# patrickltobing/shallow-wavenet

Measured on AMD Instinct MI355X. Metric: decoded samples/sec (22.05 kHz Laplacian AR decode, whole job), higher is better.
Workload: dtype f32

## Files before the change

shallow_wavenet_amd/csrc/swn_decode_bl6w.hip:

```cpp
#include <type_traits>
#include "swn_decode_bl6_common.hpp"
#include "swn_decode_internal.hpp"

namespace {

using namespace swn_bl6;

constexpr int NG = 256;
constexpr int S = 128;
constexpr int O1 = 128;

template <int LPC_, bool EXT_>
struct Tw {
    static constexpr int LPC = LPC_;
    static constexpr bool EXT = EXT_;
    using Ext = Tw<LPC_, true>;
    static constexpr int NO = 2 + LPC_;
    static constexpr int WN = cmax(1, LPC_) + 1;
    static constexpr int ring_len(int l) { return pow2ceil((1 << l) + 1); }
    static constexpr int ring_off(int l) { int o = 0; for (int i = 0; i < l; ++i) o += ring_len(i) * H; return o; }
    static constexpr int PF = L * 2 * H;
    static constexpr int NZC = 64, NZB = 4;
    static constexpr int o_ring = 0;
    static constexpr int o_hcat = o_ring + ring_off(L);
    static constexpr int o_gp = o_hcat + L * H;
    static constexpr int o_bx = o_gp + 2 * PF;
    static constexpr int o_bd = o_bx + L * 2 * H;
    static constexpr int o_old = o_bd + L * 2 * H;
    static constexpr int o_wup = o_old + 2 * L * 2 * H;
    static constexpr int o_skip = o_wup + 256;
    static constexpr int o_p2 = o_skip + S;
    static constexpr int o_tnz = o_p2 + 4 * NO;
    static constexpr int o_cz = o_tnz + r4(NZB * NZC);
    static constexpr int o_w2 = o_cz + 5 * H;
    static constexpr int o_bias = o_w2 + NO * S + r4(NO);
    static constexpr int o_w1 = o_bias + S + O1;
    static constexpr int o_wl = o_w1 + 8 * O1 * 16;
    static constexpr int o_h0w = o_wl + 8 * NG * 4;
    static constexpr int o_end = o_h0w + 3 * H;
    static constexpr size_t lds_bytes = (size_t)o_end * sizeof(float);
    static constexpr int sess_old = ring_off(L);
    static constexpr int sess_win = sess_old + 2 * L * 2 * H;
    static constexpr int sess_floats = sess_win + r4(WN);
};

__device__ __forceinline__ float sum_quads(float v) {
    v += dpp_f<0x124>(v);
    v += dpp_f<0x128>(v);
    float w = v;
    asm("s_nop 1\n\tv_permlane16_swap_b32 %0, %1" : "+v"(v), "+v"(w));
    v += w;
    w = v;
    asm("s_nop 1\n\tv_permlane32_swap_b32 %0, %1" : "+v"(v), "+v"(w));
    return v + w;
}
__device__ __forceinline__ float quad_sum_by_parity(float own, float other) {
    float s = own + dpp_f<0xB1>(other);
    s += dpp_f<0x4E>(s);
    return s;
}
template <class T, int LAYER>
__device__ __forceinline__ void layer_a(float* lds, const float (&w)[2][16], const int q, const float wj, const int pb, const int po,
                                        const int ta, const float* xr) {
    const int o = ta >> 2, p = ta & 3, pr = p & 1;
    const float e_old = lds[T::o_old + po + LAYER * 2 * H + pr * H + o];
    const float e_gx = fmaf(wj, lds[T::o_gp + pb + LAYER * 2 * H + pr * H + o], lds[T::o_bx + LAYER * 2 * H + pr * H + o]);
    const float e_hp = xr[o];
    float az = 0.f, ac = 0.f;
#pragma unroll
    for (int m = 0; m < 4; ++m) {
        const float4 x = *reinterpret_cast<const float4*>(xr + 16 * p + 4 * m);
        az = fmaf(w[0][4 * m], x.x, az); ac = fmaf(w[1][4 * m], x.x, ac);
        az = fmaf(w[0][4 * m + 1], x.y, az); ac = fmaf(w[1][4 * m + 1], x.y, ac);
        az = fmaf(w[0][4 * m + 2], x.z, az); ac = fmaf(w[1][4 * m + 2], x.z, ac);
        az = fmaf(w[0][4 * m + 3], x.w, az); ac = fmaf(w[1][4 * m + 3], x.w, ac);
    }
    const float sq = quad_sum_by_parity(pr ? ac : az, pr ? az : ac);
    __builtin_amdgcn_sched_barrier(0);
    if (p < 2) {
        const float sa = sq + e_old;
        const float v = e_gx * sa;
        const float e = exp_c(p == 0 ? -v : -2.f * fminf(fabsf(v), 64.f));
        const float r = rcp_c(1.f + e);
        const float res = p == 0 ? r : copysignf((1.f - e) * r, v);
        const float c = dpp_f<0xF5>(res);
        if (p == 0) {
            const float hn = (1.f - res) * c + res * e_hp;
            if (LAYER + 1 < L) {
                constexpr int R2 = T::ring_len(LAYER + 1 < L ? LAYER + 1 : LAYER);
                lds[T::o_ring + T::ring_off(LAYER + 1 < L ? LAYER + 1 : LAYER) + (q & (R2 - 1)) * H + o] = hn;
            }
            lds[T::o_hcat + LAYER * H + o] = hn;
        }
    }
    __builtin_amdgcn_sched_barrier(0);
}

template <class T, int LAYER, int MB = 4>
__device__ __forceinline__ void older_sum(const float* lds, const float (&w)[2][16], const int qn, const int tb, float& az, float& ac) {
    constexpr int dil = 1 << LAYER;
    constexpr int R = T::ring_len(LAYER);
    const int p = tb & 3;
    const float* ring = lds + T::o_ring + T::ring_off(LAYER);
    az = 0.f; ac = 0.f;
#pragma unroll
    for (int m = 0; m < 4; ++m) {
        const float4 x = *reinterpret_cast<const float4*>(ring + ((qn - dil) & (R - 1)) * H + 16 * p + 4 * m);
        float4 w0, w1;
        if (LAYER < L - 1) {
            w0 = make_float4(w[0][4 * m], w[0][4 * m + 1], w[0][4 * m + 2], w[0][4 * m + 3]);
            w1 = make_float4(w[1][4 * m], w[1][4 * m + 1], w[1][4 * m + 2], w[1][4 * m + 3]);
        } else {
            w0 = *reinterpret_cast<const float4*>(lds + T::o_wl + (m * NG + tb) * 4);
            w1 = *reinterpret_cast<const float4*>(lds + T::o_wl + ((4 + m) * NG + tb) * 4);
        }
        az = fmaf(w0.x, x.x, az); ac = fmaf(w1.x, x.x, ac);
        az = fmaf(w0.y, x.y, az); ac = fmaf(w1.y, x.y, ac);
        az = fmaf(w0.z, x.z, az); ac = fmaf(w1.z, x.z, ac);
        az = fmaf(w0.w, x.w, az); ac = fmaf(w1.w, x.w, ac);
        if (MB < 4 && m % MB == MB - 1) __builtin_amdgcn_sched_barrier(0);
    }
    az = sum4(az); ac = sum4(ac);
}
template <class T, int LAYER>
__device__ __forceinline__ void older_store(float* lds, const int qn, const int tb, const float az, const float ac) {
    const int o = tb >> 2, p = tb & 3, pr = p & 1;
    lds[T::o_old + (qn & 1) * (L * 2 * H) + LAYER * 2 * H + pr * H + o] = (p == 0 ? az : ac) + lds[T::o_bd + LAYER * 2 * H + pr * H + o];
}
template <class T, int LAYER, int MB = 4>
__device__ __forceinline__ void older_b(float* lds, const float (&w)[2][16], const int qn, const int tb) {
    float az, ac;
    older_sum<T, LAYER, MB>(lds, w, qn, tb, az, ac);
    if ((tb & 3) < 2) older_store<T, LAYER>(lds, qn, tb, az, ac);
}
template <class T>
__device__ __forceinline__ void older_last_rows(const float* lds, const int qn, const int tb, float4 (&x)[2], float4 (&w)[2][2]) {
    constexpr int LAYER = L - 1, dil = 1 << LAYER, R = T::ring_len(LAYER);
    const float* row = lds + T::o_ring + T::ring_off(LAYER) + ((qn - dil) & (R - 1)) * H + 16 * (tb & 3);
#pragma unroll
    for (int m = 0; m < 2; ++m) {
        x[m] = *reinterpret_cast<const float4*>(row + 4 * m);
        w[m][0] = *reinterpret_cast<const float4*>(lds + T::o_wl + (m * NG + tb) * 4);
        w[m][1] = *reinterpret_cast<const float4*>(lds + T::o_wl + ((4 + m) * NG + tb) * 4);
    }
}
template <class T>
__device__ __forceinline__ void older_last_x(float* lds, const float4 (&xe)[2], const float4 (&we)[2][2], const int qn, const int tb) {
    constexpr int LAYER = L - 1, dil = 1 << LAYER, R = T::ring_len(LAYER);
    const float* row = lds + T::o_ring + T::ring_off(LAYER) + ((qn - dil) & (R - 1)) * H + 16 * (tb & 3);
    float az = 0.f, ac = 0.f;
#pragma unroll
    for (int m = 0; m < 4; ++m) {
        float4 x, w0, w1;
        if (m < 2) { x = xe[m]; w0 = we[m][0]; w1 = we[m][1]; }
        else {
            x = *reinterpret_cast<const float4*>(row + 4 * m);
            w0 = *reinterpret_cast<const float4*>(lds + T::o_wl + (m * NG + tb) * 4);
            w1 = *reinterpret_cast<const float4*>(lds + T::o_wl + ((4 + m) * NG + tb) * 4);
        }
        az = fmaf(w0.x, x.x, az); ac = fmaf(w1.x, x.x, ac);
        az = fmaf(w0.y, x.y, az); ac = fmaf(w1.y, x.y, ac);
        az = fmaf(w0.z, x.z, az); ac = fmaf(w1.z, x.z, ac);
        az = fmaf(w0.w, x.w, az); ac = fmaf(w1.w, x.w, ac);
        if (m == 1) __builtin_amdgcn_sched_barrier(0);
    }
    az = sum4(az); ac = sum4(ac);
    if ((tb & 3) < 2) older_store<T, LAYER>(lds, qn, tb, az, ac);
}
template <int... LS> struct Layers {};
template <class T, int NW, int... LS>
__device__ __forceinline__ void older_bn(Layers<LS...>, float* lds, const float (&w)[NW][2][16], const int qn, const int tb) {
    static_assert(((LS < NW) && ...), "register-resident halves only");
    float az[sizeof...(LS)], ac[sizeof...(LS)];
    int k = 0;
    ((older_sum<T, LS>(lds, w[LS], qn, tb, az[k], ac[k]), ++k), ...);
    if ((tb & 3) < 2) {
        k = 0;
        ((older_store<T, LS>(lds, qn, tb, az[k], ac[k]), ++k), ...);
    }
}

template <class T, int LAYER>
__device__ __forceinline__ void older_rows(const float* lds, const int qn, const int tb, float4 (&x)[4]) {
    constexpr int dil = 1 << LAYER;
    constexpr int R = T::ring_len(LAYER);
    const float* row = lds + T::o_ring + T::ring_off(LAYER) + ((qn - dil) & (R - 1)) * H + 16 * (tb & 3);
#pragma unroll
    for (int m = 0; m < 4; ++m) x[m] = *reinterpret_cast<const float4*>(row + 4 * m);
}
__device__ __forceinline__ void older_sum_x(const float (&w)[2][16], const float4 (&x)[4], float& az, float& ac) {
    az = 0.f; ac = 0.f;
#pragma unroll
    for (int m = 0; m < 4; ++m) {
        az = fmaf(w[0][4 * m], x[m].x, az); ac = fmaf(w[1][4 * m], x[m].x, ac);
        az = fmaf(w[0][4 * m + 1], x[m].y, az); ac = fmaf(w[1][4 * m + 1], x[m].y, ac);
        az = fmaf(w[0][4 * m + 2], x[m].z, az); ac = fmaf(w[1][4 * m + 2], x[m].z, ac);
        az = fmaf(w[0][4 * m + 3], x[m].w, az); ac = fmaf(w[1][4 * m + 3], x[m].w, ac);
    }
    az = sum4(az); ac = sum4(ac);
}
template <class T, int... LS>
__device__ __forceinline__ void older_rows_n(Layers<LS...>, const float* lds, const int qn, const int tb, float4 (&x)[sizeof...(LS)][4]) {
    int k = 0;
    ((older_rows<T, LS>(lds, qn, tb, x[k]), ++k), ...);
}
template <class T, int NW, int... LS>
__device__ __forceinline__ void older_bn_x(Layers<LS...>, float* lds, const float (&w)[NW][2][16], const float4 (&x)[sizeof...(LS)][4],
                                           const int qn, const int tb) {
    static_assert(((LS < NW) && ...), "register-resident halves only");
    float az[sizeof...(LS)], ac[sizeof...(LS)];
    int k = 0;
    ((older_sum_x(w[LS], x[k], az[k], ac[k]), ++k), ...);
    if ((tb & 3) < 2) {
        k = 0;
        ((older_store<T, LS>(lds, qn, tb, az[k], ac[k]), ++k), ...);
    }
}

template <int LAYER>
__device__ __forceinline__ void skip_issue_b(__amdgpu_buffer_rsrc_t wsk2, float4 (&wsl)[8], const int tb, const unsigned step0) {
    const int r = tb >> 2, hp = tb & 3;
#pragma unroll
    for (int ps = 0; ps < 2; ++ps)
#pragma unroll
        for (int mm = 0; mm < 4; ++mm)
            wsl[ps * 4 + mm] = buf_ld4(wsk2, (unsigned)((r + 64 * ps) * 4 + hp) * 16u, (unsigned)((LAYER * 4 + mm) * S) * 64u + step0);
}
template <class T, int LAYER>
__device__ __forceinline__ void skip_roll_b(const float* lds, __amdgpu_buffer_rsrc_t wsk2, float4 (&wsl)[8], float (&sacc)[2], const int tb,
                                            const unsigned step0) {
    static_assert(LAYER >= 1 && LAYER < L, "slice LAYER - 1 in flight, slice LAYER to request");
    const int r = tb >> 2, hp = tb & 3;
    float4 xs[4];
#pragma unroll
    for (int mm = 0; mm < 4; ++mm) xs[mm] = *reinterpret_cast<const float4*>(lds + T::o_hcat + (LAYER - 1) * H + 16 * mm + 4 * hp);
#pragma unroll
    for (int mm = 0; mm < 4; ++mm) {
#pragma unroll
        for (int ps = 0; ps < 2; ++ps) {
            const float4 x = xs[mm], w = wsl[ps * 4 + mm];
            sacc[ps] = fmaf(w.x, x.x, sacc[ps]); sacc[ps] = fmaf(w.y, x.y, sacc[ps]);
            sacc[ps] = fmaf(w.z, x.z, sacc[ps]); sacc[ps] = fmaf(w.w, x.w, sacc[ps]);
        }
        __builtin_amdgcn_sched_barrier(0);
#pragma unroll
        for (int ps = 0; ps < 2; ++ps)
            wsl[ps * 4 + mm] = buf_ld4(wsk2, (unsigned)((r + 64 * ps) * 4 + hp) * 16u, (unsigned)((LAYER * 4 + mm) * S) * 64u + step0);
        __builtin_amdgcn_sched_barrier(0);
    }
    asm volatile("" : "+v"(sacc[0]), "+v"(sacc[1]));
}
template <class T>
__device__ __forceinline__ void skip_last_b(float* lds, const float4 (&wsl)[8], const float (&sacc)[2], const int tb) {
    const int r = tb >> 2, hp = tb & 3;
    float part[2][4];
#pragma unroll
    for (int mm = 0; mm < 4; ++mm) {
        const float4 x = *reinterpret_cast<const float4*>(lds + T::o_hcat + (L - 1) * H + 16 * mm + 4 * hp);
#pragma unroll
        for (int ps = 0; ps < 2; ++ps) {
            const float4 w = wsl[ps * 4 + mm];
            part[ps][mm] = fmaf(w.w, x.w, fmaf(w.z, x.z, fmaf(w.y, x.y, w.x * x.x)));
        }
    }
    float s[2];
#pragma unroll
    for (int ps = 0; ps < 2; ++ps) s[ps] = sacc[ps] + ((part[ps][0] + part[ps][1]) + (part[ps][2] + part[ps][3]));
    const float t0 = s[0] + dpp_f<0xB1>(s[0]), t1 = s[1] + dpp_f<0xB1>(s[1]);
    const float v = (hp < 2 ? t0 : t1) + dpp_f<0x4E>(hp < 2 ? t1 : t0);
    if ((hp & 1) == 0) lds[T::o_skip + r + 32 * hp] = fmaxf(v, 0.f);
}

using OlderMerged = Layers<3, 4>;
using OlderOut1 = Layers<0, 1, 2>;

template <class T, bool GA, bool STREAM, bool POOL = false>
__device__ __forceinline__ void decode_body(const Bl6Args& a, float* lds) {
    constexpr bool EXT = T::EXT;
    static_assert(!STREAM || EXT, "streamed chunks run the extended mode");
    constexpr bool grpA = GA;
    const int tid = threadIdx.x, b = POOL ? 0 : blockIdx.x;
    __builtin_assume(GA ? tid < NG : tid >= NG);
    const int tg = tid & (NG - 1);
    const float* __restrict__ P = a.P;
    const int U = a.U;
    const int s0 = STREAM ? a.step0 : 0;
    const bool resume = STREAM && a.resume;
    const int fb0 = STREAM ? s0 / U : 0;

    for (int e = tid; e < T::o_end; e += NT) lds[e] = 0.f;
    __syncthreads();
    for (int e = tid; e < L * 2 * H; e += NT) {
        lds[T::o_bx + e] = P[a.y.bx + e];
        const float bd = P[a.y.bd + e];
        lds[T::o_bd + e] = bd;
        lds[T::o_old + e] = bd;
    }
    for (int e = tid; e < U; e += NT) lds[T::o_wup + e] = P[a.y.wup + e];
    for (int e = tid; e < H; e += NT) lds[T::o_cz + e] = P[a.y.cb + e];
    for (int e = tid; e < S; e += NT) lds[T::o_bias + e] = P[a.y.bsk + e];
    for (int e = tid; e < O1; e += NT) lds[T::o_bias + S + e] = P[a.y.b1 + e];
    for (int e = tid; e < 2 * H; e += NT) { lds[T::o_cz + H + e] = P[a.y.cv + e]; lds[T::o_cz + 3 * H + e] = P[a.y.cc + e]; }
    for (int e = tid; e < T::NO * S; e += NT) lds[T::o_w2 + e] = P[a.y.w2 + (size_t)(e / S) * r4(S) + (e % S)];
    for (int e = tid; e < T::NO; e += NT) lds[T::o_w2 + T::NO * S + e] = P[a.y.b2 + e];
    for (int e = tid; e < 8 * O1 * 16; e += NT) lds[T::o_w1 + e] = P[a.y.w12 + e];
    const __amdgpu_buffer_rsrc_t condr =
        make_rsrc(a.cond + (size_t)b * a.Tf * a.N, (unsigned)((size_t)a.Tf * a.N * sizeof(float)));
    auto load_frame = [&](int fr) {
        float* dst = lds + T::o_gp + (fr & 1) * T::PF;
#pragma unroll
        for (int it = 0; it < (T::PF / 4 + NT - 1) / NT; ++it) {
            const int e4 = it * NT + tid;
            if (e4 < T::PF / 4)
                *reinterpret_cast<float4*>(dst + 4 * e4) =
                    buf_ld4(condr, (unsigned)tid * 16u, (unsigned)(fr * a.N * 4 + it * NT * 16));
        }
    };
    for (int fr = fb0; fr < fb0 + 2 && fr < a.Tf; ++fr) load_frame(fr);
    constexpr int NWR = grpA ? L : L - 1;
    float wreg[NWR][2][16];
    {
        const int o = tg >> 2, p = tg & 3, k = grpA ? 1 : 0;
#pragma unroll
        for (int l = 0; l < L; ++l)
#pragma unroll
            for (int r = 0; r < 2; ++r) {
                const float4* src = reinterpret_cast<const float4*>(P + a.y.wd + (((size_t)l * 2 * H + o + r * H) * 2 + k) * H + 16 * p);
#pragma unroll
                for (int v = 0; v < 4; ++v) {
                    const float4 t = src[v];
                    if (l == L - 1 && !grpA) {
                        *reinterpret_cast<float4*>(lds + T::o_wl + ((r * 4 + v) * NG + tg) * 4) = t;
                    } else {
                        float (&wr)[16] = wreg[l < NWR ? l : 0][r];
                        wr[4 * v] = t.x; wr[4 * v + 1] = t.y; wr[4 * v + 2] = t.z; wr[4 * v + 3] = t.w;
                    }
                }
            }
    }
    __syncthreads();
    const float* sess_b = STREAM ? a.sess + (size_t)b * T::sess_floats : nullptr;
    int tcp = tid;
    asm volatile("" : "+v"(tcp));
    if (resume) {
        for (int e = tcp; e < T::ring_off(L); e += NT) lds[T::o_ring + e] = sess_b[e];
        for (int e = tcp; e < 2 * L * 2 * H; e += NT) lds[T::o_old + e] = sess_b[T::sess_old + e];
        __syncthreads();
    }

    int fb = fb0, tb0 = fb0 * U;
    const int n_pro = RF;
    auto cond_taps = [&](int q, float& wj, int& pb) {
        const int t0 = q - RF;
        const int tlo = t0 < 0 ? 0 : t0;
        if (tlo >= tb0 + U) {
            fb += 1; tb0 += U;
            if (fb + 1 < a.Tf) load_frame(fb + 1);
        }
        int rel = tlo - tb0;
        int fsel = fb;
        if (rel >= U) { rel -= U; fsel = fb + 1; }
        rel = rel < U ? rel : U - 1;
        wj = lds[T::o_wup + rel];
        pb = (fsel & 1) * T::PF;
    };

    auto input_seed = [&](int q) {
        if (tid < H) {
            const int o = tid;
            float acc = c_b;
#pragma unroll
            for (int k = 0; k < 2; ++k) {
                const int r = q - (1 - k);
                if (r >= 0) acc += fmaf(k ? c_v1 : c_v0, 0.f, k ? c_c1 : c_c0);
            }
            lds[T::o_ring + (q & 1) * H + o] = ssign(acc);
        }
    };
    float win[T::WN];
#pragma unroll
    for (int k = 0; k < T::WN; ++k) win[k] = 0.f;
    if (EXT && a.seed) win[T::WN - 1] = reinterpret_cast<const float*>(a.seed)[b];
    if (resume) {
#pragma unroll
        for (int k = 0; k < T::WN; ++k) win[k] = sess_b[T::sess_win + k];
    }
    const int wv = __builtin_amdgcn_readfirstlane(tg >> 6);
    float kcb = 0.f, kv0 = 0.f, kv1 = 0.f, kc0 = 0.f, kc1 = 0.f;
    if (grpA) { const int o = tg & (H - 1); kcb = c_b; kv0 = c_v0; kv1 = c_v1; kc0 = c_c0; kc1 = c_c1; }
    auto h0_row = [&](int qn) -> int {
        return wv == 0 ? T::o_ring + (qn & 1) * H : T::o_h0w + (wv - 1) * H;
    };
    auto input_gen = [&](int row) {
        if constexpr (grpA) {
            float acc = kcb;
            acc += fmaf(kv0, win[T::WN - 2], kc0);
            acc += fmaf(kv1, win[T::WN - 1], kc1);
            lds[row + (tg & (H - 1))] = ssign(acc);
            lds_fence_compiler();
        }
    };
    float e_next = 0.f;
    auto noise_load = [&](int c) {
        const int step = c * T::NZC + tid - 64;
        if (step < a.n_steps) e_next = a.noise[(size_t)b * a.n_steps + step];
    };
    auto noise_chunk = [&](int c) {
        if (grpA && tid >= 64 && tid < 128) {
            const int k = tid - 64, step = c * T::NZC + k;
            if (step < a.n_steps) {
                const float e = EXT ? swn_noise_laplace_at(a.nz, b, step, s0 + step, 0, a.n_steps, 1) : e_next;
                const float sg = (e > 0.f) ? 1.f : ((e < 0.f) ? -1.f : 0.f);
                lds[T::o_tnz + (c & (T::NZB - 1)) * T::NZC + k] = sg * log1pf(-2.f * fabsf(e));
            }
            if (!EXT) noise_load(c + 1);
        }
    };
    if (!EXT && grpA && tid >= 64 && tid < 128) noise_load(0);
    noise_chunk(0);
    noise_chunk(1);

    const __amdgpu_buffer_rsrc_t wsk2 = make_rsrc(P + a.y.wsk2, (unsigned)(L * S * 64 * sizeof(float)));

#ifdef SWN_STAMP
    unsigned long long tw[9] = {0, 0, 0, 0, 0, 0, 0, 0, 0}, tv[6] = {0, 0, 0, 0, 0, 0}, tstep = 0, tlast = 0, tbeg = 0;
#define SWN_BAR(k) { tw[k] += __builtin_amdgcn_s_memtime() - tlast; lds_barrier(); tlast = __builtin_amdgcn_s_memtime(); }
#define SWN_WAIT_STAMP(k) { asm volatile("" :: "v"(wsl[0].x)); tv[k] += __builtin_amdgcn_s_memtime() - tlast; }
#define SWN_PRE(k) { tw[k] += __builtin_amdgcn_s_memtime() - tlast; asm volatile("s_waitcnt lgkmcnt(0)" ::: "memory"); }
#define SWN_BAR_KEEP(k, N) { lds_barrier_keep<N>(); tlast = __builtin_amdgcn_s_memtime(); }
#else
#define SWN_BAR(k) lds_barrier();
#define SWN_WAIT_STAMP(k)
#define SWN_PRE(k)
#define SWN_BAR_KEEP(k, N) lds_barrier_keep<N>();
#endif
#define SWN_PHASE_WORK(LAYER, GEN, X0)                                                                                \
    if constexpr (grpA) layer_a<T, LAYER>(lds, wreg[LAYER], q, wj, pb, po, tg,                                         \
                                          LAYER == 0 ? (X0) : lds + T::o_ring + T::ring_off(LAYER) +                   \
                                                                  (q & (T::ring_len(LAYER) - 1)) * H);                 \
    else {                                                                                                             \
        if (GEN) {    \
                      \
                      \
            if (LAYER == 0) skip_issue_b<0>(wsk2, wsl, tg, step0);                                                     \
            else { SWN_WAIT_STAMP(LAYER > 0 ? LAYER - 1 : 0) skip_roll_b<T, (LAYER > 0 ? LAYER : 1)>(lds, wsk2, wsl, sacc, tg, step0); } \
            __builtin_amdgcn_sched_barrier(0);                                                                         \
        }                                                                                                              \
        if (!(GEN)) older_b<T, LAYER>(lds, wreg[LAYER < NWR ? LAYER : 0], q + 1, tg);                                  \
        else if (LAYER == 0) older_bn<T>(OlderMerged{}, lds, wreg, q + 1, tg);                                         \
        __builtin_amdgcn_sched_barrier(0);                                                                             \
    }
#define SWN_PHASE(LAYER, GEN, X0) SWN_PHASE_WORK(LAYER, GEN, X0) if (GEN) { SWN_BAR(LAYER) } else lds_barrier();

#pragma unroll 1
    for (int q = resume ? n_pro : 0; q < n_pro; ++q) {
        float wj; int pb;
        float4 wsl[8]; float sacc[2]; const unsigned step0 = 0;
        cond_taps(q, wj, pb);
        const int po = (q & 1) * (L * 2 * H);
        input_seed(q);
        lds_barrier();
        const float* x0 = lds + T::o_ring + (q & 1) * H;
        SWN_PHASE(0, false, x0) SWN_PHASE(1, false, x0) SWN_PHASE(2, false, x0) SWN_PHASE(3, false, x0)
        SWN_PHASE(4, false, x0) SWN_PHASE(5, false, x0)
        (void)wsl; (void)sacc; (void)step0;
    }

    int rel_c = s0 - fb0 * U;
    bool fill_c = false;
    float wj_c = 0.f;
    int pb_c = 0, po_c = 0, x0_c = 0;
    auto taps_ahead = [&](int qn) {
        wj_c = lds[T::o_wup + rel_c];
        pb_c = (fb & 1) * T::PF;
        po_c = (qn & 1) * (L * 2 * H);
        x0_c = h0_row(qn);
        asm volatile("" : "+s"(pb_c), "+s"(po_c), "+s"(x0_c));
    };
    auto frame_advance = [&]() {
        rel_c += 1;
        const bool cross = rel_c >= U;
        if (cross) { rel_c = 0; fb += 1; }
        fill_c = cross && fb + 1 < a.Tf;
    };
    if constexpr (grpA) taps_ahead(RF + s0);
    input_gen(x0_c);
#ifdef SWN_STAMP
    tlast = tbeg = __builtin_amdgcn_s_memtime();
#endif
    auto gen_step = [&](const int i) __attribute__((always_inline)) {
        const int q = RF + s0 + i;
        const float wj = wj_c;
        const int pb = pb_c, po = po_c;
        if constexpr (grpA) {
            if (fill_c) load_frame(fb + 1);
        }
        float4 wsl[8];
        float sacc[2] = {0.f, 0.f};
        if constexpr (!grpA) {
            const float bs0 = lds[T::o_bias + (tg >> 2)], bs1 = lds[T::o_bias + (tg >> 2) + 64];
            if ((tg & 3) == 0) { sacc[0] = bs0; sacc[1] = bs1; }
        }
        unsigned step0 = 0;
        asm volatile("" : "+s"(step0));
        const float* x0 = lds + x0_c;
        SWN_PHASE(0, true, x0) SWN_PHASE(1, true, x0) SWN_PHASE(2, true, x0) SWN_PHASE(3, true, x0)
        SWN_PHASE(4, true, x0)
        constexpr bool EARLY5 = T::LPC == 0;
        float4 xl[2], wl[2][2];
        SWN_PHASE_WORK(5, true, x0)
        if constexpr (grpA && EARLY5) {
            SWN_PRE(5)
            lds_fence_compiler();
            __builtin_amdgcn_sched_barrier(0);
            older_last_rows<T>(lds, q + 1, tg + (int)step0, xl, wl);
            __builtin_amdgcn_sched_barrier(0);
            SWN_BAR_KEEP(5, 6)
        } else {
            SWN_BAR(5)
        }
        constexpr bool ROLL1 = T::LPC == 0;
        float4 xo[3][4];
        float4 w1e[2][2];
        if constexpr (!grpA) {
            SWN_WAIT_STAMP(5) skip_last_b<T>(lds, wsl, sacc, tg);
            SWN_PRE(6)
            lds_fence_compiler();
            __builtin_amdgcn_sched_barrier(0);
            older_rows_n<T>(OlderOut1{}, lds, q + 1, tg, xo);
            __builtin_amdgcn_sched_barrier(0);
            SWN_BAR_KEEP(6, 12)
        } else {
            if constexpr (EARLY5) older_last_x<T>(lds, xl, wl, q + 1, tg + (int)step0);
            else older_b<T, L - 1, 2>(lds, wreg[L - 1], q + 1, tg + (int)step0);
            if constexpr (ROLL1) {
                SWN_PRE(6)
                lds_fence_compiler();
                __builtin_amdgcn_sched_barrier(0);
#pragma unroll
                for (int mm = 0; mm < 2; ++mm)
#pragma unroll
                    for (int r = 0; r < 2; ++r)
                        w1e[mm][r] = *reinterpret_cast<const float4*>(lds + T::o_w1 + ((mm * O1 + (tg >> 2) + 64 * r) * 4 + (tg & 3)) * 4);
                __builtin_amdgcn_sched_barrier(0);
                SWN_BAR_KEEP(6, 4)
            } else {
                SWN_BAR(6)
            }
        }
        if constexpr (grpA) {
            const int hr = tg >> 2, hp = tg & 3;
            float a0 = 0.f, a1 = 0.f, b0 = 0.f, b1 = 0.f;
            auto X = [&](int mm) { return *reinterpret_cast<const float4*>(lds + T::o_skip + 16 * mm + 4 * hp); };
            auto W = [&](int mm, int r) { return *reinterpret_cast<const float4*>(lds + T::o_w1 + ((mm * O1 + hr + 64 * r) * 4 + hp) * 4); };
            auto fma8 = [&](int mm, const float4& x0, const float4& w0, const float4& w1) {
                float& acc = (mm & 1) ? a1 : a0;
                float& bcc = (mm & 1) ? b1 : b0;
                acc = fmaf(w0.x, x0.x, acc); acc = fmaf(w0.y, x0.y, acc); acc = fmaf(w0.z, x0.z, acc); acc = fmaf(w0.w, x0.w, acc);
                bcc = fmaf(w1.x, x0.x, bcc); bcc = fmaf(w1.y, x0.y, bcc); bcc = fmaf(w1.z, x0.z, bcc); bcc = fmaf(w1.w, x0.w, bcc);
            };
            float e_b1[2] = {0.f, 0.f}, e_w2[2] = {0.f, 0.f}, e_b2 = 0.f;
            const int e_kc = hp < T::NO ? hp : T::NO - 1;
            if constexpr (ROLL1) {
                static_assert(T::NO <= 4, "one round of out_2 rows");
                float4 xr[3] = {X(0), X(1), X(2)};
                __builtin_amdgcn_sched_barrier(0);
#pragma unroll
                for (int mm = 0; mm < 8; ++mm) {
                    fma8(mm, xr[mm % 3], w1e[mm % 2][0], w1e[mm % 2][1]);
                    __builtin_amdgcn_sched_barrier(0);
                    if (mm + 2 < 8) { w1e[mm % 2][0] = W(mm + 2, 0); w1e[mm % 2][1] = W(mm + 2, 1); }
                    if (mm + 3 < 8) xr[mm % 3] = X(mm + 3);
                    if (mm == 5) {
                        e_b1[0] = lds[T::o_bias + S + hr]; e_b1[1] = lds[T::o_bias + S + hr + 64];
                        e_w2[0] = lds[T::o_w2 + e_kc * S + hr]; e_w2[1] = lds[T::o_w2 + e_kc * S + hr + 64];
                    }
                    if (mm == 6) e_b2 = lds[T::o_w2 + T::NO * S + e_kc];
                    __builtin_amdgcn_sched_barrier(0);
                }
            } else {
#pragma unroll
                for (int mm = 0; mm < 8; ++mm) {
                    fma8(mm, X(mm), W(mm, 0), W(mm, 1));
                    if ((mm & 3) == 3) __builtin_amdgcn_sched_barrier(0);
                }
            }
            const float v = sum4(a0 + a1), u = sum4(b0 + b1);
            if constexpr (ROLL1) {
                const float o1a = fmaxf(v + e_b1[0], 0.f), o1b = fmaxf(u + e_b1[1], 0.f);
                const float pz = sum_quads(fmaf(e_w2[1], o1b, fmaf(e_w2[0], o1a, tg < 4 ? e_b2 : 0.f)));
                if ((tg & 63) < 4 && hp < T::NO) lds[T::o_p2 + 4 * hp + wv] = pz;
            } else {
                const float o1a = fmaxf(v + lds[T::o_bias + S + hr], 0.f), o1b = fmaxf(u + lds[T::o_bias + S + hr + 64], 0.f);
#pragma unroll
                for (int j = 0; j < (T::NO + 3) / 4; ++j) {
                    const int k = hp + 4 * j, kc = k < T::NO ? k : T::NO - 1;
                    const float* w2 = lds + T::o_w2 + kc * S;
                    const float b2 = lds[T::o_w2 + T::NO * S + kc];
                    const float pz = sum_quads(fmaf(w2[hr + 64], o1b, fmaf(w2[hr], o1a, tg < 4 ? b2 : 0.f)));
                    if ((tg & 63) < 4 && k < T::NO) lds[T::o_p2 + 4 * k + wv] = pz;
                }
            }
        } else {
            older_bn_x<T>(OlderOut1{}, lds, wreg, xo, q + 1, tg);
        }
        SWN_BAR(7)
        if constexpr (grpA) {
            const int ln = tg & 63;
            float tz = 0.f;
            if constexpr (!EXT) tz = lds[T::o_tnz + (i & (T::NZB * T::NZC - 1))];
            float fv = 0.f;
            if (a.forced) fv = reinterpret_cast<const float*>(a.forced)[(size_t)b * a.n_steps + i];
            const float4 pz = *reinterpret_cast<const float4*>(lds + T::o_p2 + 4 * (ln < T::NO ? ln : T::NO - 1));
            __builtin_amdgcn_sched_barrier(0);
            frame_advance();
            taps_ahead(q + 1);
            __builtin_amdgcn_sched_barrier(0);
            const float acc = (pz.x + pz.y) + (pz.z + pz.w);
            float o2[T::NO];
#pragma unroll
            for (int k = 0; k < T::NO; ++k) o2[k] = __builtin_bit_cast(float, __builtin_amdgcn_readlane(__builtin_bit_cast(int, acc), k));
            float sv;
            {
#pragma clang fp contract(off)
                const float mu = o2[0];
                const float bsc = sigm(o2[1]);
                float lpv = 0.f;
#pragma unroll
                for (int k = 0; k < T::LPC; ++k) lpv += o2[2 + T::LPC - 1 - k] * win[T::WN - T::LPC + k];
                const float t = bsc * (EXT ? lds[T::o_tnz + ((i >> 6) & (T::NZB - 1)) * T::NZC + (i & (T::NZC - 1))] : tz);
                sv = (T::LPC > 0) ? (lpv + mu) - t : mu - t;
                sv = fminf(fmaxf(sv, -1.f), 1.f);
                float fd = a.forced ? fv : sv;
                asm volatile("" : "+v"(fd));
#pragma unroll
                for (int k = 0; k + 1 < T::WN; ++k) win[k] = win[k + 1];
                win[T::WN - 1] = fd;
            }
            if (i + 1 < a.n_steps) input_gen(x0_c);
            __builtin_amdgcn_sched_barrier(0);
            if (tid == 0) reinterpret_cast<float*>(a.out)[(size_t)b * a.n_steps + (size_t)i] = sv;
            if (HEADS_ON && a.heads && wv == 0 && ln < T::NO) a.heads[((size_t)b * a.n_steps + i) * T::NO + ln] = acc;
        }
#ifdef SWN_STAMP
        if constexpr (grpA) tw[8] += __builtin_amdgcn_s_memtime() - tlast;
#endif
    };
#pragma unroll 1
    for (int i0 = 0; i0 < a.n_steps; i0 += T::NZC) {
        noise_chunk((i0 >> 6) + 2);
        const int iend = i0 + T::NZC < a.n_steps ? i0 + T::NZC : a.n_steps;
#pragma unroll 1
        for (int i = i0; i < iend; ++i) gen_step(i);
    }
#ifdef SWN_STAMP
    { const unsigned long long tn = __builtin_amdgcn_s_memtime(); tw[0] += tn - tlast; tstep = tn - tbeg; }
#endif
    if constexpr (STREAM) {
        __syncthreads();
        float* so = a.sess + (size_t)b * T::sess_floats;
        tcp = tid;
        asm volatile("" : "+v"(tcp));
        for (int e = tcp; e < T::ring_off(L); e += NT) so[e] = lds[T::o_ring + e];
        for (int e = tcp; e < 2 * L * 2 * H; e += NT) so[T::sess_old + e] = lds[T::o_old + e];
        if (tid == 0) {
#pragma unroll
            for (int k = 0; k < T::WN; ++k) so[T::sess_win + k] = win[k];
        }
    }
#undef SWN_PHASE
#undef SWN_PHASE_WORK
#undef SWN_BAR
#undef SWN_WAIT_STAMP
#undef SWN_PRE
#undef SWN_BAR_KEEP
#ifdef SWN_STAMP
    if ((tid == 0 || tid == 64 || tid == NG) && b == 0 && a.heads) {
        float* h = a.heads + (tid == 0 ? 0 : tid == 64 ? 30 : 10);
        for (int k = 0; k < 9; ++k) h[k] = (float)((double)tw[k] / (double)a.n_steps);
        if (tid == 0) h[9] = (float)((double)tstep / (double)a.n_steps);
        else if (tid == NG) for (int k = 0; k < 6; ++k) h[10 + k] = (float)((double)tv[k] / (double)a.n_steps);
    }
#endif
}

template <class T, bool STREAM = false>
__global__ __launch_bounds__(NT) void decode_bl6w_kernel(const Bl6Args a) {
    extern __shared__ __attribute__((aligned(16))) float lds[];
    if (threadIdx.x < NG) decode_body<T, true, STREAM>(a, lds);
    else decode_body<T, false, STREAM>(a, lds);
}

template <class T, bool MODELS = false>
__global__ __launch_bounds__(NT) void decode_bl6w_pool_kernel(
    const typename std::conditional<MODELS, Bl6PoolModelsArgs, Bl6PoolArgs>::type p) {
    extern __shared__ __attribute__((aligned(16))) float lds[];
    static_assert(T::EXT, "pools run the extended mode");
    Bl6Args a = p.c;
    if constexpr (MODELS) a.P = swn_pool_model(p.m);
    if (!swn_pool_entry_args(a, p.t, 1, 1, T::NO)) return;
    a.sess += (size_t)swn_pool_slot(p.t) * T::sess_floats;
    if (threadIdx.x < NG) decode_body<T, true, true, true>(a, lds);
    else decode_body<T, false, true, true>(a, lds);
}

bool bl6w_applies(const SwnGeom& g) {
    return g.bl6 && g.U <= 256 && g.U >= 2 && !g.audio_in && g.kind == SWN_KIND_LAPLACE && g.S == 128 && g.O1 == 128 &&
           g.seg == 1 && (g.lpc == 0 || g.lpc == 4);
}

template <class F>
int with_tw(const SwnGeom& g, F&& f) {
    if (!bl6w_applies(g)) return SWN_E_UNSUPPORTED;
    if (g.lpc == 0) return f(Tw<0, false>{});
    return f(Tw<4, false>{});
}

}

int swn_decode_bl6w_run(const SwnDecodeCall& c) {
    const hipStream_t st = c.hip_stream;
    if (c.pool) {
        Bl6PoolModelsArgs p;
        fill_args(p.c, c);
        p.t = *c.pool;
        if (c.models) p.m = *c.models;
        return with_tw(c.g, [&](auto tw) {
            using T = typename decltype(tw)::Ext;
            if (c.models)
                return launch_kernel(decode_bl6w_pool_kernel<T, true>, T::lds_bytes, c.batch, p, st, "swn_decode_pool_chunk_models(bl6w)");
            const Bl6PoolArgs& p1 = p;
            return launch_kernel(decode_bl6w_pool_kernel<T>, T::lds_bytes, c.batch, p1, st, "swn_decode_pool_chunk(bl6w)");
        });
    }
    Bl6Args a;
    fill_args(a, c);
    return with_tw(c.g, [&](auto t) {
        using T = decltype(t);
        using X = typename T::Ext;
        static_assert(T::lds_bytes <= 160 * 1024 && X::lds_bytes <= 160 * 1024, "LDS budget");
        if (c.stream) return launch_kernel(decode_bl6w_kernel<X, true>, X::lds_bytes, a.B, a, st, "swn_decode(bl6w)");
        if (wants_ext(a)) return launch_kernel(decode_bl6w_kernel<X>, X::lds_bytes, a.B, a, st, "swn_decode(bl6w)");
        return launch_kernel(decode_bl6w_kernel<T>, T::lds_bytes, a.B, a, st, "swn_decode(bl6w)");
    });
}

size_t swn_decode_bl6w_session_floats(const SwnGeom& g) {
    int n = 0;
    with_tw(g, [&](auto t) { n = decltype(t)::sess_floats; return SWN_OK; });
    return (size_t)n;
}
```

Baseline: 395,200.

## Rotate per-step side work behind layer-0 LDS loads and keep one skip slice resident

In the non-extended, LPC==0 path, group A now issues the first quads of layer-0 LDS input loads and then runs the per-step side work while those loads are in flight. That side work is the noise-chunk refresh, the frame load and a deferred buffer store of the previous step's output and heads. The step loop is flattened so noise refresh happens inside the step. Group B can optionally keep the first or last skip-weight slice resident in registers so one global reload per step is skipped; this is controlled by a macro whose default is off. The aim is to hide LDS and store latency on the serial decode critical path, at the cost of more registers and output writes that lag by one step.

```diff
diff --git a/shallow_wavenet_amd/csrc/swn_decode_bl6w.hip b/shallow_wavenet_amd/csrc/swn_decode_bl6w.hip
--- a/shallow_wavenet_amd/csrc/swn_decode_bl6w.hip
+++ b/shallow_wavenet_amd/csrc/swn_decode_bl6w.hip
@@ -1,6 +1,13 @@
 #include <type_traits>
 #include "swn_decode_bl6_common.hpp"
 #include "swn_decode_internal.hpp"
+
+#ifndef SWN_RES_SLICE
+#define SWN_RES_SLICE 0
+#endif
+#ifndef SWN_ROTATE
+#define SWN_ROTATE 1
+#endif
 
 namespace {
 
@@ -59,17 +66,31 @@
     s += dpp_f<0x4E>(s);
     return s;
 }
-template <class T, int LAYER>
+struct NoWork { __device__ __forceinline__ void operator()() const {} };
+template <class T, int LAYER, int NQ = 2, class BEHIND = NoWork>
 __device__ __forceinline__ void layer_a(float* lds, const float (&w)[2][16], const int q, const float wj, const int pb, const int po,
-                                        const int ta, const float* xr) {
+                                        const int ta, const float* xr, BEHIND&& behind = NoWork{}) {
+    constexpr bool ROT = !std::is_same<typename std::decay<BEHIND>::type, NoWork>::value;
     const int o = ta >> 2, p = ta & 3, pr = p & 1;
     const float e_old = lds[T::o_old + po + LAYER * 2 * H + pr * H + o];
-    const float e_gx = fmaf(wj, lds[T::o_gp + pb + LAYER * 2 * H + pr * H + o], lds[T::o_bx + LAYER * 2 * H + pr * H + o]);
+    const float g_gp = lds[T::o_gp + pb + LAYER * 2 * H + pr * H + o], g_bx = lds[T::o_bx + LAYER * 2 * H + pr * H + o];
     const float e_hp = xr[o];
+    static_assert(NQ >= 0 && NQ <= 4, "early quads");
+    float4 xq[4];
+    if constexpr (ROT) {
+#pragma unroll
+        for (int m = 0; m < NQ; ++m) xq[m] = *reinterpret_cast<const float4*>(xr + 16 * p + 4 * m);
+        __builtin_amdgcn_sched_barrier(0);
+        behind();
+        __builtin_amdgcn_sched_barrier(0);
+    }
+    const float e_gx = fmaf(wj, g_gp, g_bx);
     float az = 0.f, ac = 0.f;
 #pragma unroll
     for (int m = 0; m < 4; ++m) {
-        const float4 x = *reinterpret_cast<const float4*>(xr + 16 * p + 4 * m);
+        float4 x;
+        if (ROT && m < NQ) x = xq[m];
+        else x = *reinterpret_cast<const float4*>(xr + 16 * p + 4 * m);
         az = fmaf(w[0][4 * m], x.x, az); ac = fmaf(w[1][4 * m], x.x, ac);
         az = fmaf(w[0][4 * m + 1], x.y, az); ac = fmaf(w[1][4 * m + 1], x.y, ac);
         az = fmaf(w[0][4 * m + 2], x.z, az); ac = fmaf(w[1][4 * m + 2], x.z, ac);
@@ -226,9 +247,9 @@
         for (int mm = 0; mm < 4; ++mm)
             wsl[ps * 4 + mm] = buf_ld4(wsk2, (unsigned)((r + 64 * ps) * 4 + hp) * 16u, (unsigned)((LAYER * 4 + mm) * S) * 64u + step0);
 }
-template <class T, int LAYER>
-__device__ __forceinline__ void skip_roll_b(const float* lds, __amdgpu_buffer_rsrc_t wsk2, float4 (&wsl)[8], float (&sacc)[2], const int tb,
-                                            const unsigned step0) {
+template <class T, int LAYER, bool REQ = true>
+__device__ __forceinline__ void skip_roll_b(const float* lds, __amdgpu_buffer_rsrc_t wsk2, const float4 (&wcur)[8], float4 (&wnext)[8],
+                                            float (&sacc)[2], const int tb, const unsigned step0) {
     static_assert(LAYER >= 1 && LAYER < L, "slice LAYER - 1 in flight, slice LAYER to request");
     const int r = tb >> 2, hp = tb & 3;
     float4 xs[4];
@@ -238,14 +259,14 @@
     for (int mm = 0; mm < 4; ++mm) {
 #pragma unroll
         for (int ps = 0; ps < 2; ++ps) {
-            const float4 x = xs[mm], w = wsl[ps * 4 + mm];
+            const float4 x = xs[mm], w = wcur[ps * 4 + mm];
             sacc[ps] = fmaf(w.x, x.x, sacc[ps]); sacc[ps] = fmaf(w.y, x.y, sacc[ps]);
             sacc[ps] = fmaf(w.z, x.z, sacc[ps]); sacc[ps] = fmaf(w.w, x.w, sacc[ps]);
         }
         __builtin_amdgcn_sched_barrier(0);
 #pragma unroll
         for (int ps = 0; ps < 2; ++ps)
-            wsl[ps * 4 + mm] = buf_ld4(wsk2, (unsigned)((r + 64 * ps) * 4 + hp) * 16u, (unsigned)((LAYER * 4 + mm) * S) * 64u + step0);
+            if (REQ) wnext[ps * 4 + mm] = buf_ld4(wsk2, (unsigned)((r + 64 * ps) * 4 + hp) * 16u, (unsigned)((LAYER * 4 + mm) * S) * 64u + step0);
         __builtin_amdgcn_sched_barrier(0);
     }
     asm volatile("" : "+v"(sacc[0]), "+v"(sacc[1]));
@@ -421,6 +442,12 @@
     noise_chunk(1);
 
     const __amdgpu_buffer_rsrc_t wsk2 = make_rsrc(P + a.y.wsk2, (unsigned)(L * S * 64 * sizeof(float)));
+    constexpr bool NEWFORM = !EXT && T::LPC == 0;
+    constexpr int RES = (grpA || !NEWFORM) ? -1 : SWN_RES_SLICE;
+    static_assert(RES == -1 || RES == 0 || RES == L - 1, "the first or the last slice");
+    float4 wres[8];
+    if constexpr (RES == 0) skip_issue_b<0>(wsk2, wres, tg, 0u);
+    if constexpr (RES == L - 1) skip_issue_b<L - 1>(wsk2, wres, tg, 0u);
 
 #ifdef SWN_STAMP
     unsigned long long tw[9] = {0, 0, 0, 0, 0, 0, 0, 0, 0}, tv[6] = {0, 0, 0, 0, 0, 0}, tstep = 0, tlast = 0, tbeg = 0;
@@ -442,8 +469,11 @@
         if (GEN) {    \
                       \
                       \
-            if (LAYER == 0) skip_issue_b<0>(wsk2, wsl, tg, step0);                                                     \
-            else { SWN_WAIT_STAMP(LAYER > 0 ? LAYER - 1 : 0) skip_roll_b<T, (LAYER > 0 ? LAYER : 1)>(lds, wsk2, wsl, sacc, tg, step0); } \
+                      \
+            if (LAYER == 0) { if (RES != 0) skip_issue_b<0>(wsk2, wsl, tg, step0); }                                   \
+            else if (LAYER == 1 && RES == 0) skip_roll_b<T, 1>(lds, wsk2, wres, wsl, sacc, tg, step0);                 \
+            else { SWN_WAIT_STAMP(LAYER > 0 ? LAYER - 1 : 0)                                                           \
+                   skip_roll_b<T, (LAYER > 0 ? LAYER : 1), !(LAYER == L - 1 && RES == L - 1)>(lds, wsk2, wsl, wsl, sacc, tg, step0); } \
             __builtin_amdgcn_sched_barrier(0);                                                                         \
         }                                                                                                              \
         if (!(GEN)) older_b<T, LAYER>(lds, wreg[LAYER < NWR ? LAYER : 0], q + 1, tg);                                  \
@@ -488,13 +518,37 @@
 #ifdef SWN_STAMP
     tlast = tbeg = __builtin_amdgcn_s_memtime();
 #endif
+    constexpr bool ROT = SWN_ROTATE && NEWFORM;
+    constexpr int ROTQ = 2;
+    float sv_p = 0.f, acc_p = 0.f;
+    const __amdgpu_buffer_rsrc_t outr =
+        make_rsrc(reinterpret_cast<float*>(a.out) + (size_t)b * a.n_steps, (unsigned)((size_t)a.n_steps * sizeof(float)));
+    const __amdgpu_buffer_rsrc_t headr =
+        make_rsrc(HEADS_ON && a.heads ? a.heads + (size_t)b * a.n_steps * T::NO : nullptr,
+                  HEADS_ON && a.heads ? (unsigned)((size_t)a.n_steps * T::NO * sizeof(float)) : 0u);
+    auto store_step = [&](const int ip) __attribute__((always_inline)) {
+        if constexpr (grpA && ROT) {
+            if (tid == 0) __builtin_amdgcn_raw_buffer_store_b32(__builtin_bit_cast(unsigned, sv_p), outr, 0u, (unsigned)ip * 4u, 0);
+            if (wv == 0 && (tg & 63) < T::NO)
+                __builtin_amdgcn_raw_buffer_store_b32(__builtin_bit_cast(unsigned, acc_p), headr, (unsigned)(tg & 63) * 4u,
+                                                      (unsigned)(ip * T::NO) * 4u, 0);
+        } else if constexpr (grpA) {
+            if (tid == 0) reinterpret_cast<float*>(a.out)[(size_t)b * a.n_steps + (size_t)ip] = sv_p;
+            if (HEADS_ON && a.heads && wv == 0 && (tg & 63) < T::NO) a.heads[((size_t)b * a.n_steps + ip) * T::NO + (tg & 63)] = acc_p;
+        }
+    };
     auto gen_step = [&](const int i) __attribute__((always_inline)) {
         const int q = RF + s0 + i;
         const float wj = wj_c;
         const int pb = pb_c, po = po_c;
-        if constexpr (grpA) {
+        if constexpr (grpA && !ROT) {
             if (fill_c) load_frame(fb + 1);
         }
+        auto behind0 = [&]() __attribute__((always_inline)) {
+            if ((i & (T::NZC - 1)) == 0) noise_chunk((i >> 6) + 2);
+            if (fill_c) load_frame(fb + 1);
+            if (i > 0) store_step(i - 1);
+        };
         float4 wsl[8];
         float sacc[2] = {0.f, 0.f};
         if constexpr (!grpA) {
@@ -504,7 +558,13 @@
         unsigned step0 = 0;
         asm volatile("" : "+s"(step0));
         const float* x0 = lds + x0_c;
-        SWN_PHASE(0, true, x0) SWN_PHASE(1, true, x0) SWN_PHASE(2, true, x0) SWN_PHASE(3, true, x0)
+        if constexpr (grpA && ROT) {
+            layer_a<T, 0, ROTQ>(lds, wreg[0], q, wj, pb, po, tg, x0, behind0);
+            SWN_BAR(0)
+        } else {
+            SWN_PHASE(0, true, x0)
+        }
+        SWN_PHASE(1, true, x0) SWN_PHASE(2, true, x0) SWN_PHASE(3, true, x0)
         SWN_PHASE(4, true, x0)
         constexpr bool EARLY5 = T::LPC == 0;
         float4 xl[2], wl[2][2];
@@ -523,7 +583,8 @@
         float4 xo[3][4];
         float4 w1e[2][2];
         if constexpr (!grpA) {
-            SWN_WAIT_STAMP(5) skip_last_b<T>(lds, wsl, sacc, tg);
+            if constexpr (RES == L - 1) skip_last_b<T>(lds, wres, sacc, tg);
+            else { SWN_WAIT_STAMP(5) skip_last_b<T>(lds, wsl, sacc, tg); }
             SWN_PRE(6)
             lds_fence_compiler();
             __builtin_amdgcn_sched_barrier(0);
@@ -639,19 +700,28 @@
             }
             if (i + 1 < a.n_steps) input_gen(x0_c);
             __builtin_amdgcn_sched_barrier(0);
-            if (tid == 0) reinterpret_cast<float*>(a.out)[(size_t)b * a.n_steps + (size_t)i] = sv;
-            if (HEADS_ON && a.heads && wv == 0 && ln < T::NO) a.heads[((size_t)b * a.n_steps + i) * T::NO + ln] = acc;
+            if constexpr (ROT) { sv_p = sv; acc_p = acc; }
+            else {
+                if (tid == 0) reinterpret_cast<float*>(a.out)[(size_t)b * a.n_steps + (size_t)i] = sv;
+                if (HEADS_ON && a.heads && wv == 0 && ln < T::NO) a.heads[((size_t)b * a.n_steps + i) * T::NO + ln] = acc;
+            }
         }
 #ifdef SWN_STAMP
         if constexpr (grpA) tw[8] += __builtin_amdgcn_s_memtime() - tlast;
 #endif
     };
+    if constexpr (ROT) {
 #pragma unroll 1
-    for (int i0 = 0; i0 < a.n_steps; i0 += T::NZC) {
-        noise_chunk((i0 >> 6) + 2);
-        const int iend = i0 + T::NZC < a.n_steps ? i0 + T::NZC : a.n_steps;
+        for (int i = 0; i < a.n_steps; ++i) gen_step(i);
+        if (a.n_steps > 0) store_step(a.n_steps - 1);
+    } else {
 #pragma unroll 1
-        for (int i = i0; i < iend; ++i) gen_step(i);
+        for (int i0 = 0; i0 < a.n_steps; i0 += T::NZC) {
+            noise_chunk((i0 >> 6) + 2);
+            const int iend = i0 + T::NZC < a.n_steps ? i0 + T::NZC : a.n_steps;
+#pragma unroll 1
+            for (int i = i0; i < iend; ++i) gen_step(i);
+        }
     }
 #ifdef SWN_STAMP
     { const unsigned long long tn = __builtin_amdgcn_s_memtime(); tw[0] += tn - tlast; tstep = tn - tbeg; }
```

New measurement: 401,200, median of 6. +1.5%, better.
